# ug93tad/singa

Hardware: AMD Instinct MI355X
Metric: images/sec (whole node) ResNet-50 bf16 training (higher is better)
Workload: dtype bf16; 1 GPU; model=ResNet-50, global_batch=1024, image=224, parallelism=dp1, exec=hipgraph, optimizer=SGD momentum 0.9 wd 1e-4, deterministic=True

## Files before the change

### singa_amd/csrc/kernels/igemm.hip

```cpp
#include <stdio.h>
#include <stdlib.h>

#include <stdexcept>
#include <type_traits>

#include "igemm_kern.h"

namespace sg {

constexpr int WDOT_RB = 64;
__global__ void __launch_bounds__(256) wdot_colsum_k(const bf16* __restrict__ w, const float* __restrict__ dw,
                                                     int rows, int C, float sign, float* __restrict__ wdot,
                                                     const float* __restrict__ gamma, const float* __restrict__ beta,
                                                     float tau, int* __restrict__ flag) {
  __shared__ float red[4][64];
  const int cl = threadIdx.x & 63, lane = threadIdx.x >> 6;
  const int c = blockIdx.x * 64 + cl;
  if (gamma != nullptr && blockIdx.y == 0 && lane == 0 && c < C) {
    const float g = fabsf(gamma[c]);
    if (!(g >= tau && fabsf(beta[c]) <= 4.f * g)) *flag = 1;
  }
  const int r0 = blockIdx.y * WDOT_RB;
  float a = 0.f;
  if (c < C) {
    const int r1 = min(rows, r0 + WDOT_RB);
    for (int r = r0 + lane; r < r1; r += 4) a += (float)w[(int64_t)r * C + c] * dw[(int64_t)r * C + c];
  }
  red[lane][cl] = a;
  __syncthreads();
  if (lane == 0 && c < C) atomicAdd(wdot + c, sign * (red[0][cl] + red[1][cl] + red[2][cl] + red[3][cl]));
}

__global__ void __launch_bounds__(256) wt_transpose_k(const bf16* __restrict__ w, bf16* __restrict__ wt, int K,
                                                      int T, int C) {
  __shared__ bf16 tile[64][65];
  const int c0 = blockIdx.x * 64, k0 = blockIdx.y * 64, t = blockIdx.z;
  const int tx = threadIdx.x & 63, ty = threadIdx.x >> 6;
  for (int r = ty; r < 64; r += 4) {
    const int k = k0 + r, c = c0 + tx;
    tile[r][tx] = (k < K && c < C) ? w[((int64_t)k * T + t) * C + c] : (bf16)0.f;
  }
  __syncthreads();
  for (int r = ty; r < 64; r += 4) {
    const int c = c0 + r, k = k0 + tx;
    if (c < C && k < K) wt[((int64_t)t * C + c) * K + k] = tile[tx][r];
  }
}

struct WtDesc {
  const bf16* src;
  bf16* dst;
  int K, T, C, tile0;
};
__global__ void __launch_bounds__(256) wt_transpose_batched_k(const WtDesc* __restrict__ desc, int n) {
  __shared__ bf16 tile[64][65];
  int d = 0;
  while (d + 1 < n && desc[d + 1].tile0 <= (int)blockIdx.x) ++d;
  const WtDesc w = desc[d];
  const int lt = blockIdx.x - w.tile0;
  const int cb = (w.C + 63) / 64, kbn = (w.K + 63) / 64;
  const int c0 = (lt % cb) * 64, k0 = ((lt / cb) % kbn) * 64, t = lt / (cb * kbn);
  const int tx = threadIdx.x & 63, ty = threadIdx.x >> 6;
  for (int r = ty; r < 64; r += 4) {
    const int k = k0 + r, c = c0 + tx;
    tile[r][tx] = (k < w.K && c < w.C) ? w.src[((int64_t)k * w.T + t) * w.C + c] : (bf16)0.f;
  }
  __syncthreads();
  for (int r = ty; r < 64; r += 4) {
    const int c = c0 + r, k = k0 + tx;
    if (c < w.C && k < w.K) w.dst[((int64_t)t * w.C + c) * w.K + k] = tile[tx][r];
  }
}

}

using namespace sg;

static void init_phase_identity(ConvGeom& g) {
  for (int i = 0; i < 16; ++i) {
    g.phs[i].dns = FastDiv(1);
    g.phs[i].dWp = FastDiv(1);
    g.phs[i].dHpWp = FastDiv(1);
  }
}

static ConvGeom make_geom(int N, int H, int W, int C, int K, int R, int S, int Ho, int Wo, int sh, int sw, int ph,
                          int pw, int dh, int dw) {
  ConvGeom g{};
  g.N = N; g.H = H; g.W = W; g.C = C; g.K = K; g.R = R; g.S = S; g.Ho = Ho; g.Wo = Wo;
  g.sh = sh; g.sw = sw; g.ph = ph; g.pw = pw; g.dh = dh; g.dw = dw;
  g.dC = FastDiv(C); g.dS = FastDiv(S); g.dK = FastDiv(K); g.dWo = FastDiv(Wo); g.dHoWo = FastDiv(Ho * Wo);
  g.bq_n = BK / (Ho * Wo);
  g.bq_h = (BK % (Ho * Wo)) / Wo;
  g.bq_w = BK % Wo;
  init_phase_identity(g);
  return g;
}

static int make_phases(ConvGeom& g) {
  int np = 0;
  for (int a = 0; a < g.sh; ++a)
    for (int b = 0; b < g.sw; ++b) {
      Phase& P = g.phs[np++];
      P.a = a; P.b = b;
      P.r0 = (a + g.ph) % g.sh;
      P.s0 = (b + g.pw) % g.sw;
      P.nr = P.r0 < g.R ? (g.R - P.r0 + g.sh - 1) / g.sh : 0;
      P.ns = P.s0 < g.S ? (g.S - P.s0 + g.sw - 1) / g.sw : 0;
      P.offh = (a + g.ph - P.r0) / g.sh;
      P.offw = (b + g.pw - P.s0) / g.sw;
      P.Hp = a < g.H ? (g.H - a + g.sh - 1) / g.sh : 0;
      P.Wp = b < g.W ? (g.W - b + g.sw - 1) / g.sw : 0;
      P.dns = FastDiv(P.ns > 0 ? P.ns : 1);
      P.dWp = FastDiv(P.Wp > 0 ? P.Wp : 1);
      P.dHpWp = FastDiv(P.Hp * P.Wp > 0 ? P.Hp * P.Wp : 1);
    }
  return np;
}

extern "C" int sg_bn_deterministic();
static int g_tune[20] = {5, 1, 1, 0, 0, 1, 2, 1, 0, 1, 0, 0, 0, 1, 0, 1, 0, 0, 1, 0};
static thread_local int g_wt_ready = 0;
static thread_local const bf16* g_res_g = nullptr;
static thread_local int g_res_s = 1, g_res_Ho = 0, g_res_Wo = 0;
static thread_local const uint8_t* g_res_mask = nullptr;
static thread_local int g_mask_out = 0;

static int gemm_log() {
  static int on = [] {
    const char* e = getenv("SG_GEMM_LOG");
    return e && e[0] == '1' ? 1 : 0;
  }();
  return on;
}

constexpr int stages_c(int BM, int BN, int STAGES) { return STAGES * (BM + BN) * BK * 2; }

template <int BM, int BN, int AM, int BMODE, int OUT, int NTH = NT, int WM = 2, int WN = 2, int STAGES = 2,
          int FLAGS = 0>
static void launch_t(const GemmArgs& p_in, int tiles, int ydim, int zdim, hipStream_t s) {
  GemmArgs p = p_in;
  p.lds_epilogue = g_tune[1];
  p.epi_fence = g_tune[19];
  p.early_issue = g_tune[7];
  p.nt_store = g_tune[8];
  p.xcd_split = (OUT == OUT_F32_ATOMIC && g_tune[2] && ydim == 1 && zdim >= 8 && (zdim & 7) == 0) ? 1 : 0;
  dim3 grid(tiles, ydim, zdim), block(NTH);
  constexpr int stages = STAGES * (BM + BN) * BK * 2;
  constexpr int rch = (STAGES == 1 || BM * (BN + 4) * 4 <= 152 * 1024) ? BM : BM / 4;
  constexpr int etile = STAGES == 1 ? (OUT == OUT_BF16 ? BM * (BN + 8) * 2 : BM * (BN + 4) * 4)
                        : OUT == OUT_BF16 ? rch * (BN + 4) * 4
                        : OUT == OUT_F32_ATOMIC ? BM * (BN + 4) * 4 : 0;
  constexpr int ered = (OUT == OUT_BF16) ? NTH * 16 * 4 : 0;
  static_assert(STAGES != 1 || (OUT == OUT_BF16 && ered <= (etile > stages_c(BM, BN, STAGES) ? etile : stages_c(BM, BN, STAGES))),
                "single-stage variant: bf16 output only");
  constexpr int lds = stages > etile ? stages : etile;
  static_assert(lds <= 160 * 1024, "LDS budget");
  auto* kern = igemm_k<BM, BN, AM, BMODE, OUT, NTH, WM, WN, STAGES, FLAGS>;
  if (gemm_log())
    fprintf(stderr, "SG_GEMM_L igemm_k<%d,%d,%d,%d,%d,%d,%d,%d,%d,%d> grid %d %d %d\n", BM, BN, AM, BMODE, OUT, NTH, WM,
            WN, STAGES, FLAGS, tiles, ydim, zdim);
  if constexpr (lds > 65536) {
    static bool attr = [kern] {
      return hipFuncSetAttribute((const void*)kern, hipFuncAttributeMaxDynamicSharedMemorySize, lds) == hipSuccess;
    }();
    (void)attr;
  }
  hipLaunchKernelGGL(kern, grid, block, lds, s, p);
}

template <int OUT, int FLAGS = 0>
static void launch_pp(const GemmArgs& p_in, int tiles, int ydim, hipStream_t s) {
  GemmArgs p = p_in;
  p.lds_epilogue = g_tune[1];
  p.epi_fence = g_tune[19];
  p.nt_store = g_tune[8];
  constexpr int lds = 2 * PP_BUF;
  auto* kern = pp_gemm_k<OUT, FLAGS>;
  if (gemm_log()) fprintf(stderr, "SG_GEMM_L pp_gemm_k<%d,%d> grid %d %d 1\n", OUT, FLAGS, tiles, ydim);
  static bool attr = [kern] {
    return hipFuncSetAttribute((const void*)kern, hipFuncAttributeMaxDynamicSharedMemorySize, lds) == hipSuccess;
  }();
  (void)attr;
  hipLaunchKernelGGL(kern, dim3(tiles, ydim, 1), dim3(512), lds, s, p);
}

template <int KT, int EPI = 0, int AM = LM_KMAJOR>
static void launch_sk(const GemmArgs& p, int tiles_m, int tiles_n, hipStream_t s) {
  constexpr int lds = sk_lds(KT);
  auto* kern = sk_gemm_k<KT, EPI, AM>;
  static bool attr = [kern] {
    return hipFuncSetAttribute((const void*)kern, hipFuncAttributeMaxDynamicSharedMemorySize, lds) == hipSuccess;
  }();
  (void)attr;
  const int cus = sg_cu_count();
  int g = (cus + tiles_n - 1) / tiles_n;
  g = (g + 7) / 8 * 8;
  if (g > tiles_m) g = tiles_m >= 8 ? tiles_m / 8 * 8 : 8;
  GemmArgs q = p;
  q.wq = 8 * tiles_n <= QMAX ? sg_workq_slot() : nullptr;
  if (gemm_log())
    fprintf(stderr, "SG_GEMM_L sk_gemm_k<%d,%d,%d> grid %d %d 1 M=%d N=%d K=%d\n", KT, EPI, AM, g, tiles_n, p.M, p.N,
            p.K);
  hipLaunchKernelGGL(kern, dim3(g, tiles_n, 1), dim3(256), lds, s, q);
}

static void launch_st(const GemmArgs& p, int tiles_m, int tiles_n, hipStream_t s) {
  auto* kern = st_gemm_k<0>;
  static bool attr = [kern] {
    return hipFuncSetAttribute((const void*)kern, hipFuncAttributeMaxDynamicSharedMemorySize, ST_LDS) == hipSuccess;
  }();
  (void)attr;
  const int cus = sg_cu_count();
  int g = (cus + tiles_n - 1) / tiles_n;
  g = (g + 7) / 8 * 8;
  if (g > tiles_m) g = tiles_m >= 8 ? tiles_m / 8 * 8 : 8;
  GemmArgs q = p;
  q.wq = 8 * tiles_n <= QMAX ? sg_workq_slot() : nullptr;
  if (gemm_log())
    fprintf(stderr, "SG_GEMM_L st_gemm_k<0> grid %d %d 1 M=%d N=%d K=%d\n", g, tiles_n, p.M, p.N, p.K);
  hipLaunchKernelGGL(kern, dim3(g, tiles_n, 1), dim3(256), ST_LDS, s, q);
}

static int pick_big(int M, int N) {
  if (g_tune[4] == 5) return 1;
  if (g_tune[4] == 6) return 2;
  if (g_tune[4] == 7) return 3;
  if (g_tune[4] == 8) return 4;
  if (!g_tune[5] || g_tune[4] != 0) return 0;
  auto wg = [&](int bm, int bn) { return (long)((M + bm - 1) / bm) * ((N + bn - 1) / bn); };
  if (N >= 128 && !((N % 128) != 0 && (N % 128) <= 64) && wg(128, 128) >= 512) return 1;
  return 0;
}
static int big_bm(int big) { return big == 1 ? 128 : 256; }

static void pick_tile(int M, int N, int& BM, int& BN) {
  auto wg = [&](int bm, int bn) { return (long)((M + bm - 1) / bm) * ((N + bn - 1) / bn); };
  BM = 128;
  BN = N <= 64 ? 64 : 128;
  if (BN == 128 && (N % 128) != 0 && (N % 128) <= 64) BN = 64;
  if (wg(BM, BN) < 256 && M > 64) BM = 64;
  if (wg(BM, BN) < 256 && BN == 128) BN = 64;
}

template <int AM, int BMODE, int OUT>
static void launch_tile(const GemmArgs& p, int M, int BM, int BN, int splits, hipStream_t s, int batch, int zdim) {
  const int tiles = ((M + BM - 1) / BM) * ((p.N + BN - 1) / BN);
  const int z = zdim > 0 ? zdim : splits;
  if (BM == 128 && BN == 128) launch_t<128, 128, AM, BMODE, OUT>(p, tiles, batch, z, s);
  else if (BM == 128 && BN == 64) launch_t<128, 64, AM, BMODE, OUT>(p, tiles, batch, z, s);
  else if (BM == 64 && BN == 128) launch_t<64, 128, AM, BMODE, OUT>(p, tiles, batch, z, s);
  else launch_t<64, 64, AM, BMODE, OUT>(p, tiles, batch, z, s);
}

static void pick_wgrad(int M, int N, int K, int mode, int& BM, int& BN, int& splits) {
  const int nkt = (K + BK - 1) / BK;
  if (mode == 4) mode = ((long)K >= 8L * M * N) ? 1 : 0;
  if (mode == 0) {
    pick_tile(M, N, BM, BN);
    const int tiles = ((M + BM - 1) / BM) * ((N + BN - 1) / BN);
    splits = 1;
    while (tiles * splits < 768 && splits * 2 <= nkt / 4) splits *= 2;
    return;
  }
  auto fit = [](int d) { return (d >= 128 && !((d % 128) != 0 && (d % 128) <= 64)) ? 128 : 64; };
  BM = fit(M);
  BN = fit(N);
  const int tiles = ((M + BM - 1) / BM) * ((N + BN - 1) / BN);
  const int target = mode == 1 ? 512 : mode == 2 ? 1024 : 768;
  const int min_kt = mode == 2 ? 4 : 8;
  splits = 1;
  while (tiles * splits < target && (splits * 2) * min_kt <= nkt) splits *= 2;
}

template <int AM, int BMODE, int OUT, int FLAGS = 0>
static void launch(const GemmArgs& p, int M, int splits, hipStream_t s, int batch, int zdim) {
  int BM, BN;
  if (gemm_log())
    fprintf(stderr, "SG_GEMM am=%d bm=%d out=%d flags=%d M=%d N=%d K=%d splits=%d batch=%d z=%d beta=%g stats=%d "
                    "smode=%d det=%d res=%d bias=%d relu=%d act=%d phase=%d R=%d S=%d C=%d sh=%d\n",
            AM, BMODE, OUT, FLAGS, M, p.N, p.K, splits, batch, zdim, p.beta, p.stats != nullptr, p.stats_mode,
            p.stats_det, p.res_g != nullptr, p.bias != nullptr, p.relu, p.act, p.out_phase, p.g.R, p.g.S, p.g.C,
            p.g.sh);
  if constexpr (OUT != OUT_F32_ATOMIC) {
    {
      const int z = zdim > 0 ? zdim : 1;
      if (FLAGS == 0 && OUT == OUT_BF16 && AM == LM_KMAJOR && BMODE == LM_KMAJOR && g_tune[9] && g_tune[4] == 0 &&
          !p.out_phase && zdim <= 1 && batch == 1 && p.K <= 128 && (p.N & 127) == 0 && !p.bias && !p.relu &&
          p.alpha == 1.f && p.stats_mode == 0 && !(p.stats && p.stats_det) && g_tune[1] && !p.res_g &&
          (p.ldc & 7) == 0 && (long)((M + 127) / 128) * (p.N / 128) >= 2048) {
        const int tiles_m = (M + 127) / 128;
        if (p.K <= 64) launch_sk<1>(p, tiles_m, p.N / 128, s);
        else launch_sk<2>(p, tiles_m, p.N / 128, s);
        return;
      }
      if (FLAGS == 0 && OUT == OUT_BF16 && AM == LM_KMAJOR && BMODE == LM_KMAJOR && g_tune[18] && g_tune[4] == 0 &&
          (g_tune[18] >= 2 || p.K == 256 || (p.K == 512 && p.N == 128)) &&
          !p.out_phase && zdim <= 1 && batch == 1 && p.K >= 256 && (p.K & 63) == 0 && (p.N & 127) == 0 &&
          !p.bias && !p.relu && p.act == 0 && p.act_bwd == 0 && p.alpha == 1.f && p.beta == 0.f &&
          p.stats_mode == 0 && !(p.stats && p.stats_det) && !p.res_g && g_tune[1] && (p.ldc & 7) == 0 &&
          (p.lda & 7) == 0 && (p.ldb & 7) == 0 && (long)((M + 127) / 128) * (p.N / 128) >= 2048) {
        launch_st(p, (M + 127) / 128, p.N / 128, s);
        return;
      }
      int kmax = p.K;
      if (p.out_phase) {
        kmax = 0;
        for (int i = 0; i < z; ++i) kmax = max(kmax, p.g.phs[i].nr * p.g.phs[i].ns * p.g.K);
      }
      if (OUT == OUT_BF16 && g_tune[6] > 0 && g_tune[4] == 0 && p.beta == 0.f &&
          (kmax + BK - 1) / BK <= g_tune[6] && p.N >= 128 && !((p.N % 128) != 0 && (p.N % 128) <= 64) &&
          (long)((M + 127) / 128) * ((p.N + 127) / 128) >= 1024 && (g_tune[11] == 0 || !p.out_phase)) {
        const int tiles = ((M + 127) / 128) * ((p.N + 127) / 128);
        launch_t<128, 128, AM, BMODE, OUT_BF16, 256, 2, 2, 1, FLAGS>(p, tiles, batch, z, s);
        return;
      }
      int big = pick_big(M, p.N);
      const bool pp_ok = AM == LM_KMAJOR && BMODE == LM_KMAJOR && !p.out_phase && zdim <= 1 &&
                         !(p.stats && p.stats_det);
      if (big == 0 && g_tune[4] == 0 && g_tune[5] && pp_ok && p.K >= 2048 &&
          (long)((M + 255) / 256) * ((p.N + 255) / 256) >= 256)
        big = 4;
      if (big == 4) {
        if (pp_ok) {
          launch_pp<OUT, FLAGS>(p, ((M + 255) / 256) * ((p.N + 255) / 256), batch, s);
          return;
        }
        big = 1;
      }
      if (big == 1 && g_tune[16] > 0 && !sg_bn_deterministic() && M >= 256 &&
          (g_tune[16] >= 3 || AM == LM_CONV_FWD || (g_tune[16] == 2 && AM == LM_DGRAD_A)))
        big = 3;
      if (big == 1) {
        const int tiles = ((M + 127) / 128) * ((p.N + 127) / 128);
        launch_t<128, 128, AM, BMODE, OUT, 512, 2, 4, 2, FLAGS>(p, tiles, batch, z, s);
        return;
      }
      if (big == 2) {
        const int tiles = ((M + 255) / 256) * ((p.N + 63) / 64);
        launch_t<256, 64, AM, BMODE, OUT, 512, 4, 2, 4, FLAGS>(p, tiles, batch, z, s);
        return;
      }
      if (big == 3) {
        const int tiles = ((M + 255) / 256) * ((p.N + 127) / 128);
        launch_t<256, 128, AM, BMODE, OUT, 512, 4, 2, 3, FLAGS>(p, tiles, batch, z, s);
        return;
      }
    }
  }
  pick_tile(M, p.N, BM, BN);
  if (g_tune[4] > 0 && g_tune[4] < 5) {
    BM = (g_tune[4] == 2 || g_tune[4] == 3) ? 64 : 128;
    BN = (g_tune[4] == 1 || g_tune[4] == 3) ? 64 : 128;
  }
  const int tiles = ((M + BM - 1) / BM) * ((p.N + BN - 1) / BN);
  const int z = zdim > 0 ? zdim : splits;
  if constexpr ((AM == LM_KMAJOR || AM == LM_KOUTER) && (BMODE == LM_KMAJOR || BMODE == LM_KOUTER) && FLAGS == 0) {
    const long wgs = (long)tiles * (batch > 0 ? batch : 1) * (z > 0 ? z : 1);
    const int nkt = ((z > 1 ? p.k_per_split : p.K) + BK - 1) / BK;
    const bool ring = g_tune[14] == 3 || (g_tune[14] == 0 && wgs <= 4L * sg_cu_count() && nkt >= 8 && nkt <= 64);
    if (ring && !p.out_phase) {
      if (BM == 128 && BN == 128) launch_t<128, 128, AM, BMODE, OUT, NT, 2, 2, 3>(p, tiles, batch, z, s);
      else if (BM == 128 && BN == 64) launch_t<128, 64, AM, BMODE, OUT, NT, 2, 2, 3>(p, tiles, batch, z, s);
      else if (BM == 64 && BN == 128) launch_t<64, 128, AM, BMODE, OUT, NT, 2, 2, 3>(p, tiles, batch, z, s);
      else launch_t<64, 64, AM, BMODE, OUT, NT, 2, 2, 3>(p, tiles, batch, z, s);
      return;
    }
  }
  if (BM == 128 && BN == 128) launch_t<128, 128, AM, BMODE, OUT, NT, 2, 2, 2, FLAGS>(p, tiles, batch, z, s);
  else if (BM == 128 && BN == 64) launch_t<128, 64, AM, BMODE, OUT, NT, 2, 2, 2, FLAGS>(p, tiles, batch, z, s);
  else if (BM == 64 && BN == 128) launch_t<64, 128, AM, BMODE, OUT, NT, 2, 2, 2, FLAGS>(p, tiles, batch, z, s);
  else launch_t<64, 64, AM, BMODE, OUT, NT, 2, 2, 2, FLAGS>(p, tiles, batch, z, s);
}

static int pick_splits(int M, int N, int K, int want) {
  if (want > 0) return want;
  int BM, BN;
  pick_tile(M, N, BM, BN);
  const int tiles = ((M + BM - 1) / BM) * ((N + BN - 1) / BN);
  int splits = 1;
  const int nkt = (K + BK - 1) / BK;
  const int cap = 2 * sg_cu_count();
  while (tiles * splits * 2 <= cap && nkt / (splits * 2) >= 32) splits *= 2;
  if (tiles < cap / 8)
    while (tiles * splits < cap && nkt / (splits * 2) >= 4) splits *= 2;
  return splits;
}

static inline int kps(int K, int splits) {
  const int nkt = (K + BK - 1) / BK;
  return ((nkt + splits - 1) / splits) * BK;
}

static unsigned extent_bytes(int64_t elems) {
  if (elems * 2 >= (int64_t)1 << 31)
    throw std::runtime_error("igemm: operand exceeds 2 GiB (32-bit buffer offsets); split the batch");
  return (unsigned)(elems * 2);
}

extern "C" {

int sg_bn_deterministic();
int sg_ws_prezeroed();
int sg_conv3x3_ok(int N, int H, int W, int C, int K);
int sg_conv3x3_64(const void* x, const void* w, int wmode, void* y, void* stats, const void* mask, int N, int H,
                  int W, int C, int K, hipStream_t s);

void sg_gemm_heads(const void* a, int64_t lda, int a_kouter, const void* b, int64_t ldb, int b_kouter, void* c,
                   int64_t ldc, int M, int N, int K, float alpha, float beta, const void* bias, int relu,
                   int out_mode, int splits, int batch, int64_t sa, int64_t sb, int64_t sc, int bh, int64_t sa2,
                   int64_t sb2, int64_t sc2, hipStream_t s);

void sg_gemm(const void* a, int64_t lda, int a_kouter, const void* b, int64_t ldb, int b_kouter, void* c,
             int64_t ldc, int M, int N, int K, float alpha, float beta, const void* bias, int relu, int out_mode,
             int splits, int batch, int64_t sa, int64_t sb, int64_t sc, hipStream_t s) {
  sg_gemm_heads(a, lda, a_kouter, b, ldb, b_kouter, c, ldc, M, N, K, alpha, beta, bias, relu, out_mode, splits,
                batch, sa, sb, sc, 0, 0, 0, 0, s);
}

int sg_gemm_act(const void* a, int64_t lda, int a_kouter, const void* b, int64_t ldb, int b_kouter, void* c,
                int64_t ldc, int M, int N, int K, float alpha, const void* bias, int batch, int64_t sa, int64_t sb,
                int64_t sc, int act, void* aux, int act_bwd, const void* act_x, float* colsum, hipStream_t s) {
  if ((N & 7) != 0 || (ldc & 7) != 0 || !g_tune[1] || g_tune[4] != 0 || (act == 0) == (act_x == nullptr) ||
      M <= 0 || K <= 0 || batch != 1 || (colsum && (act != 0 || sg_bn_deterministic())))
    return 0;
  GemmArgs p{};
  init_phase_identity(p.g);
  p.sa = sa; p.sb = sb; p.sc = sc;
  p.M = M; p.N = N; p.K = K; p.a = (const bf16*)a; p.lda = lda; p.b = (const bf16*)b; p.ldb = ldb;
  p.c = c; p.ldc = ldc; p.alpha = alpha; p.beta = 0.f; p.bias = (const float*)bias; p.relu = 0;
  p.act = act; p.aux = (bf16*)aux; p.act_x = (const bf16*)act_x; p.act_bwd = act_bwd;
  if (colsum) {
    p.stats = colsum;
    p.stats_mode = 5;
    p.stats_det = 0;
  }
  p.k_per_split = kps(K, 1);
  p.a_bytes = extent_bytes(a_kouter ? (int64_t)(K - 1) * lda + M : (int64_t)(M - 1) * lda + K);
  p.b_bytes = extent_bytes(b_kouter ? (int64_t)(K - 1) * ldb + N : (int64_t)(N - 1) * ldb + K);
// ... 224 lines not shown
    if (wt && (K & 63) == 0) {
      if (!wt_ready)
        hipLaunchKernelGGL(wt_transpose_k, dim3((C + 63) / 64, (K + 63) / 64, 1), dim3(256), 0, s, (const bf16*)w,
                           (bf16*)wt, K, 1, C);
      p.b = (const bf16*)wt; p.ldb = K;
      if (p.stats && p.stats_mode == 4 && p.res_s <= 1 && out_mode == OUT_BF16 && beta == 0.f && g_tune[9] &&
          g_tune[4] == 0 && K <= 128 && (C & 127) == 0 && (long)((p.M + 127) / 128) * (C / 128) >= 2048) {
        GemmArgs q = p;
        q.ep_res = p.res_g;
        q.ep_mask = (uint8_t*)p.bnb_mask;
        q.res_g = nullptr;
        if (K <= 64) launch_sk<1, 2>(q, (p.M + 127) / 128, C / 128, s);
        else launch_sk<2, 2>(q, (p.M + 127) / 128, C / 128, s);
        return;
      }
      if (out_mode == OUT_F32) launch<LM_KMAJOR, LM_KMAJOR, OUT_F32>(p, p.M, 1, s, 1, 0);
      else launch<LM_KMAJOR, LM_KMAJOR, OUT_BF16>(p, p.M, 1, s, 1, 0);
    } else {
      p.b = (const bf16*)w; p.ldb = C;
      if (out_mode == OUT_F32) launch<LM_KMAJOR, LM_KOUTER, OUT_F32>(p, p.M, 1, s, 1, 0);
      else launch<LM_KMAJOR, LM_KOUTER, OUT_BF16>(p, p.M, 1, s, 1, 0);
    }
    return;
  }
  const int np = make_phases(p.g);
  int Mmax = 0;
  for (int i = 0; i < np; ++i) Mmax = Mmax > N * p.g.phs[i].Hp * p.g.phs[i].Wp ? Mmax : N * p.g.phs[i].Hp * p.g.phs[i].Wp;
  p.M = Mmax; p.N = C; p.K = R * S * K;
  p.a = (const bf16*)dy; p.lda = 0; p.b = (const bf16*)w; p.ldb = 0;
  p.c = dx; p.ldc = C; p.alpha = 1.f; p.beta = beta; p.bias = nullptr; p.relu = 0;
  p.out_phase = 1;
  p.k_per_split = kps(p.K, 1);
  p.a_bytes = extent_bytes((int64_t)N * Ho * Wo * K);
  p.b_bytes = extent_bytes((int64_t)K * R * S * C);
  extent_bytes((int64_t)N * H * W * C);
  if (wt && (K & 63) == 0) {
    if (!wt_ready)
      hipLaunchKernelGGL(wt_transpose_k, dim3((C + 63) / 64, (K + 63) / 64, R * S), dim3(256), 0, s, (const bf16*)w,
                         (bf16*)wt, K, R * S, C);
    p.b = (const bf16*)wt;
    if (out_mode == OUT_F32) launch<LM_DGRAD_A, LM_DGRAD_BT, OUT_F32>(p, Mmax, 1, s, 1, np);
    else launch<LM_DGRAD_A, LM_DGRAD_BT, OUT_BF16>(p, Mmax, 1, s, 1, np);
    return;
  }
  if (out_mode == OUT_F32) launch<LM_DGRAD_A, LM_DGRAD_B, OUT_F32>(p, Mmax, 1, s, 1, np);
  else launch<LM_DGRAD_A, LM_DGRAD_B, OUT_BF16>(p, Mmax, 1, s, 1, np);
}

static int wgrad_splits_q(int tiles, int nkt, int sp0, int per_cu = 2) {
  const int slots = per_cu * sg_cu_count();
  constexpr int e = 6;
  int best = sp0;
  long best_cost = (long)((tiles * sp0 + slots - 1) / slots) * ((nkt + sp0 - 1) / sp0 + e);
  for (int sp = 1; sp <= 2 * sp0 && nkt / sp >= 16; ++sp) {
    const long cost = (long)((tiles * sp + slots - 1) / slots) * ((nkt + sp - 1) / sp + e);
    if (cost < best_cost || (cost == best_cost && sp < best)) {
      best = sp;
      best_cost = cost;
    }
  }
  return best;
}

void sg_conv_wgrad(const void* x, const void* dy, void* dw_out, int N, int H, int W, int C, int K, int R, int S,
                   int Ho, int Wo, int sh, int sw, int ph, int pw, int dh, int dw, int splits, hipStream_t s) {
  GemmArgs p{};
  p.g = make_geom(N, H, W, C, K, R, S, Ho, Wo, sh, sw, ph, pw, dh, dw);
  p.M = K; p.N = R * S * C; p.K = N * Ho * Wo;
  p.a = (const bf16*)dy; p.lda = K; p.b = (const bf16*)x; p.ldb = 0;
  p.c = dw_out; p.ldc = R * S * C; p.alpha = 1.f; p.beta = 0.f; p.bias = nullptr; p.relu = 0;
  p.a_bytes = extent_bytes((int64_t)N * Ho * Wo * K);
  p.b_bytes = extent_bytes((int64_t)N * H * W * C);
  int BM, BN, sp;
  int mode = g_tune[0], extra = g_tune[3];
  if (mode == 5) {
    if (R * S > 1) {
      mode = 4;
      extra += K <= 128 ? 2 : 1;
    } else {
      mode = (sh > 1 || sw > 1 || C == 2 * K) ? 1 : 4;
    }
  }
  pick_wgrad(p.M, p.N, p.K, mode, BM, BN, sp);
  if (extra > 0) {
    const int nkt = (p.K + BK - 1) / BK;
    for (int i = 0; i < extra && sp * 2 <= nkt; ++i) sp *= 2;
  }
  const bool big = g_tune[5] && p.M >= 128 && p.N >= 128 && splits <= 0 && !sg_bn_deterministic();
  if (big) {
    const int tiles = ((p.M + 127) / 128) * ((p.N + 127) / 128);
    const int nkt = (p.K + BK - 1) / BK;
    const int target = g_tune[10] > 0 ? g_tune[10] : R * S > 1 ? 1024 : 512;
    sp = 1;
    while (tiles * sp < target && sp * 2 * 4 <= nkt) sp *= 2;
    if (g_tune[13] && g_tune[10] <= 0) sp = wgrad_splits_q(tiles, nkt, sp);
    if (g_tune[12] > 0) sp = g_tune[12];
    if (g_tune[15] == 1 && p.M >= 256 && (p.M & 255) == 0) {
      const int t2 = ((p.M + 255) / 256) * ((p.N + 127) / 128);
      int sp2 = 1;
      while (t2 * sp2 < target && sp2 * 2 * 4 <= nkt) sp2 *= 2;
      if (g_tune[13] && g_tune[10] <= 0) sp2 = wgrad_splits_q(t2, nkt, sp2, 1);
      if (g_tune[12] > 0) sp2 = g_tune[12];
      p.k_per_split = kps(p.K, sp2);
      launch_t<256, 128, LM_KOUTER, LM_WGRAD_B, OUT_F32_ATOMIC, 512, 4, 2, 3>(p, t2, 1, sp2, s);
      return;
    }
    if (g_tune[15] == 1 && g_tune[17] == 1 && p.M < 256 && p.N >= 256) {
      const int t2 = ((p.M + 127) / 128) * ((p.N + 255) / 256);
      int sp2 = 1;
      while (t2 * sp2 < target && sp2 * 2 * 4 <= nkt) sp2 *= 2;
      if (g_tune[13] && g_tune[10] <= 0) sp2 = wgrad_splits_q(t2, nkt, sp2, 1);
      if (g_tune[12] > 0) sp2 = g_tune[12];
      p.k_per_split = kps(p.K, sp2);
      launch_t<128, 256, LM_KOUTER, LM_WGRAD_B, OUT_F32_ATOMIC, 512, 2, 4, 3>(p, t2, 1, sp2, s);
      return;
    }
    p.k_per_split = kps(p.K, sp);
    launch_t<128, 128, LM_KOUTER, LM_WGRAD_B, OUT_F32_ATOMIC, 512, 2, 4, 2>(p, tiles, 1, sp, s);
    return;
  }
  if (splits > 0) sp = splits;
  if (sg_bn_deterministic()) sp = 1;
  p.k_per_split = kps(p.K, sp);
  launch_tile<LM_KOUTER, LM_WGRAD_B, OUT_F32_ATOMIC>(p, p.M, BM, BN, sp, s, 1, 0);
}

int sg_conv_stats_rows(int M, int N) {
  if ((N & 7) != 0 || !g_tune[1]) return 0;
  if (!sg_bn_deterministic()) return 32;
  if (int big = pick_big(M, N)) {
    if (big == 4) big = 1;
    return (M + big_bm(big) - 1) / big_bm(big);
  }
  int BM, BN;
  pick_tile(M, N, BM, BN);
  return (M + BM - 1) / BM;
}

void sg_set_wt_ready(int on) { g_wt_ready = on; }
void sg_set_dgrad_mask_out(int on) { g_mask_out = on; }
void sg_wdot_colsum(const void* w, const void* dw, int rows, int C, float sign, void* wdot, int zero_first,
                    const void* gamma, const void* beta, float tau, hipStream_t s) {
  if (zero_first && !sg_ws_prezeroed()) sg_zero_async(wdot, sizeof(float) * (C + 1), s);
  hipLaunchKernelGGL(wdot_colsum_k, dim3((C + 63) / 64, (rows + WDOT_RB - 1) / WDOT_RB), dim3(256), 0, s,
                     (const bf16*)w, (const float*)dw, rows, C, sign, (float*)wdot, (const float*)gamma,
                     (const float*)beta, tau, (int*)((float*)wdot + C));
}
void sg_wt_transpose_batched(const void* desc, int n, int total, hipStream_t s) {
  static_assert(sizeof(WtDesc) == 32, "descriptor layout shared with the Python packer");
  if (n > 0 && total > 0)
    hipLaunchKernelGGL(wt_transpose_batched_k, dim3(total), dim3(256), 0, s, (const WtDesc*)desc, n);
}
void sg_set_tuning(int key, int value) {
  if (key >= 0 && key < 20) g_tune[key] = value;
}
int sg_get_tuning(int key) { return key >= 0 && key < 20 ? g_tune[key] : 0; }

}
```

### singa_amd/csrc/kernels/igemm_kern.h

```cpp
#pragma once
#include <stdexcept>
#include <type_traits>

#include "common.h"

namespace sg {

constexpr int BK = 64, NT = 256;

enum LoadMode : int {
  LM_KMAJOR = 0,
  LM_KOUTER = 1,
  LM_CONV_FWD = 2,
  LM_DGRAD_A = 3,
  LM_WGRAD_B = 4,
  LM_DGRAD_B = 5,
  LM_DGRAD_BT = 6,
  LM_KMAJOR2 = 7,
  LM_KOUTER2 = 8,
};
enum OutMode : int { OUT_BF16 = 0, OUT_F32 = 1, OUT_F32_ATOMIC = 2 };

struct Phase {
  int a, b;
// ... 977 lines not shown
      else if constexpr (EPI == 2) wait_vmcnt<5 * NPS + D + 1>();
      else if (has_beta) wait_vmcnt<2 * NPS + D + 1>(); else wait_vmcnt<NPS + D + 1>();
    } else {
      if constexpr (EPI >= 1) wait_vmcnt<6 * NPS + D + 1>();
      else if (has_beta) wait_vmcnt<4 * NPS + D + 1>(); else wait_vmcnt<2 * NPS + D + 1>();
    }
    raw_barrier();
    f32x4 acc[TM][TN];
#pragma unroll
    for (int i = 0; i < TM; ++i)
#pragma unroll
      for (int j = 0; j < TN; ++j) acc[i][j] = f32x4{0.f, 0.f, 0.f, 0.f};
#pragma unroll
    for (int kt = 0; kt < KT; ++kt) {
      const char* a_img = sA + (buf * KT + kt) * SK_TILE;
      const char* b_img = sB + kt * SK_TILE;
#pragma unroll
      for (int kk = 0; kk < 2; ++kk) {
        bf16x8 fa[TM], fb[TN];
#pragma unroll
        for (int i = 0; i < TM; ++i) fa[i] = la.frag_at(a_img, oa0[i][kk], oa1[i][kk]);
#pragma unroll
        for (int j = 0; j < TN; ++j) fb[j] = lb.frag_at(b_img, ob0[j][kk], ob1[j][kk]);
#pragma unroll
        for (int i = 0; i < TM; ++i)
#pragma unroll
          for (int j = 0; j < TN; ++j)
            acc[i][j] = __builtin_amdgcn_mfma_f32_16x16x32_bf16(fb[j], fa[i], acc[i][j], 0, 0, 0);
      }
    }
#pragma unroll
    for (int i = 0; i < TM; ++i) {
      const int ml = wm * WTM + i * 16 + (l & 15);
#pragma unroll
      for (int j = 0; j < TN; ++j) {
        const int nl = wn * WTN + j * 16 + (l >> 4) * 4;
        bf16x4 o;
        o[0] = (bf16)acc[i][j][0]; o[1] = (bf16)acc[i][j][1]; o[2] = (bf16)acc[i][j][2]; o[3] = (bf16)acc[i][j][3];
        *(bf16x4*)(sC + ml * SK_LDT + nl) = o;
      }
    }
    if (it > 0 && wid == 0 && l == 0) {
      if constexpr (EPI >= 1) wait_vmcnt<3 * NPS + D>();
      else if (has_beta) wait_vmcnt<2 * NPS + D>(); else wait_vmcnt<NPS + D>();
      *sQ =p.wq ? xcd + 8 * (3 * G8 + ticket) : tm + 16 * G8;
    }
    __builtin_amdgcn_s_waitcnt(0xC07F);
    raw_barrier();
    if (it > 0) t2 = __builtin_amdgcn_readfirstlane(*sQ);
    queue_op();
    {
      const bool live = t2 < tiles_m;
      la.init(p, (live ? t2 : tm) * BM, M, P, p.lda, p.a, p.a_bytes);
#pragma unroll
      for (int kt = 0; kt < KT; ++kt) la.issue(p, t2 * BM, M, kt * BK, K, P, sA + (buf * KT + kt) * SK_TILE, live);
    }
    const int m0 = tm * BM;
    const int rows = min(BM, M - m0);
    const __amdgpu_buffer_rsrc_t rc =
        p.c ? make_rsrc((const bf16*)p.c + (int64_t)m0 * p.ldc, (unsigned)((int64_t)rows * p.ldc * 2)) : rnull;
    u32x4 old[NPS];
    if constexpr (EPI == 1) {
      const __amdgpu_buffer_rsrc_t rmk = make_rsrc(p.ep_mask + (int64_t)m0 * (N >> 3), (unsigned)(rows * (N >> 3)));
#pragma unroll
      for (int pass = 0; pass < NPS; ++pass) {
        const int ml = r0 + pass * RPP;
        bf16x8 o = *(const bf16x8*)(sC + ml * SK_LDT + ch * 8);
        const bf16x8 rb = __builtin_bit_cast(bf16x8, rres[pass]);
        unsigned b = 0;
#pragma unroll
        for (int r = 0; r < 8; ++r) {
          o[r] = (bf16)fmaxf((float)o[r] * esc[r] + esf[r] + (float)rb[r], 0.f);
          b |= ((float)o[r] > 0.f ? 1u : 0u) << r;
        }
        __builtin_amdgcn_raw_buffer_store_b128(__builtin_bit_cast(u32x4, o), rc, (unsigned)((ml * (int)p.ldc + n) * 2),
                                               0, 0);
        __builtin_amdgcn_raw_buffer_store_b8((unsigned char)b, rmk, (unsigned)(ml * (N >> 3) + (n >> 3)), 0, 0);
      }
      load_res(t1);
    } else if constexpr (EPI == 2) {
#pragma unroll
      for (int pass = 0; pass < NPS; ++pass) {
        const int ml = r0 + pass * RPP;
        bf16x8 o = *(const bf16x8*)(sC + ml * SK_LDT + ch * 8);
        const bf16x8 rb = __builtin_bit_cast(bf16x8, rres[pass]);
#pragma unroll
        for (int r = 0; r < 8; ++r)
          o[r] = ((mres[pass] >> r) & 1u) != 0 ? (bf16)((float)o[r] + (float)rb[r]) : (bf16)0.f;
        __builtin_amdgcn_raw_buffer_store_b128(__builtin_bit_cast(u32x4, o), rc, (unsigned)((ml * (int)p.ldc + n) * 2),
                                               0, 0);
        if (ml < rows) {
#pragma unroll
          for (int r = 0; r < 8; ++r) st_s[r] += (float)o[r];
        }
      }
      load_res(t1);
    } else {
      if (has_beta) {
#pragma unroll
        for (int pass = 0; pass < NPS; ++pass)
          old[pass] = __builtin_amdgcn_raw_buffer_load_b128(rc, (unsigned)(((r0 + pass * RPP) * (int)p.ldc + n) * 2), 0, 0);
      }
#pragma unroll
      for (int pass = 0; pass < NPS; ++pass) {
        const int ml = r0 + pass * RPP;
        bf16x8 o = *(const bf16x8*)(sC + ml * SK_LDT + ch * 8);
        if (has_beta) {
          const bf16x8 ob = __builtin_bit_cast(bf16x8, old[pass]);
#pragma unroll
          for (int r = 0; r < 8; ++r) o[r] = (bf16)((float)o[r] + p.beta * (float)ob[r]);
        }
        __builtin_amdgcn_raw_buffer_store_b128(__builtin_bit_cast(u32x4, o), rc, (unsigned)((ml * (int)p.ldc + n) * 2),
                                               0, 0);
        if (p.stats && ml < rows) {
#pragma unroll
          for (int r = 0; r < 8; ++r) {
            const float f = (float)o[r];
            st_s[r] += f;
            st_q[r] += f * f;
          }
        }
      }
    }
    tm = t1;
    t1 = t2;
    if (tm >= tiles_m) break;
  }
  wait_vmcnt<0>();
  if (p.wq && threadIdx.x == 0) wq_done(p.wq, 8 * (int)gridDim.y);
  if (EPI != 1 && p.stats) {
    __syncthreads();
    float* red = (float*)smem;
#pragma unroll
    for (int r = 0; r < 8; ++r) {
      red[threadIdx.x * 16 + r] = st_s[r];
      red[threadIdx.x * 16 + 8 + r] = st_q[r];
    }
    __syncthreads();
    if (threadIdx.x < CPRW * 16) {
      const int c = threadIdx.x >> 4, r = threadIdx.x & 15;
      const int nn = n0 + c * 8;
      if (nn < N) {
        float a = red[c * 16 + r];
        for (int k = 1; k < RPP; ++k) a += red[(k * CPRW + c) * 16 + r];
        const int col = r < 8 ? nn + r : N + nn + (r - 8);
        atomicAdd(p.stats + (int64_t)(blockIdx.x & 31) * 2 * N + col, a);
      }
    }
  }
}

constexpr int ST_STAGE = 2 * SK_TILE;

__device__ __forceinline__ int wq_take_nowait(int* slot, int q) {
  int v;
  int* addr = slot + q * QSTRIDE;
  asm volatile("global_atomic_add %0, %1, %2, off sc0" : "=v"(v) : "v"(addr), "v"(1) : "memory");
  return v;
}
constexpr int ST_LDS = 3 * ST_STAGE + SK_STG;

template <int EPI = 0>
__global__ void __launch_bounds__(256, 1) st_gemm_k(const GemmArgs p) {
  extern __shared__ __attribute__((aligned(16))) char smem[];
  constexpr int BM = 128, BN = 128, NTH = 256, WN = 2, WTM = 64, WTN = 64, TM = 4, TN = 4;
  static_assert(EPI == 0, "plain output with optional BN statistics");
  bf16* sC = (bf16*)(smem + 3 * ST_STAGE);
  int* sQ = (int*)(smem + ST_LDS - 16);
  const int M = p.M, N = p.N, K = p.K;
  const int KT = K / BK;
  const int tiles_m = (M + BM - 1) / BM;
  const int n0 = blockIdx.y * BN;
  const int G = (int)gridDim.x, G8 = G >> 3, xcd = blockIdx.x & 7;
  const int qid = blockIdx.y * 8 + xcd;
  int tm = xcd + 8 * (blockIdx.x >> 3);
  int t1 = tm + 8 * G8, t2 = tm + 16 * G8;
  const Phase& P = p.g.phs[0];
  const int l = threadIdx.x & 63;
  const int wid = threadIdx.x >> 6;
  const int wm = wid / WN, wn = wid % WN;
  if (tm >= tiles_m) {
    if (p.wq && threadIdx.x == 0) wq_done(p.wq, 8 * (int)gridDim.y);
    return;
  }
  Loader<BM, LM_KMAJOR, NTH> la, la1;
  Loader<BN, LM_KMAJOR, NTH> lb;
  lb.init(p, n0, N, P, p.ldb, p.b, p.b_bytes);
  la.init(p, tm * BM, M, P, p.lda, p.a, p.a_bytes);
  la1.init(p, (t1 < tiles_m ? t1 : tm) * BM, M, P, p.lda, p.a, p.a_bytes);
  constexpr int LPT = Loader<BM, LM_KMAJOR, NTH>::VPT + Loader<BN, LM_KMAJOR, NTH>::VPT;
  constexpr int CPRW = BN / 8, RPP = NTH / CPRW, NPS = BM / RPP;
  constexpr int E_OPS = NPS + 1;
  static_assert(2 * LPT + E_OPS < 64, "vmcnt range");
  auto issue = [&](Loader<BM, LM_KMAJOR, NTH>& a, int t, int kt, int st) {
    char* base = smem + st * ST_STAGE;
    const bool live = t < tiles_m;
    a.issue(p, t * BM, M, kt * BK, K, P, base, live);
    lb.issue(p, n0, N, kt * BK, K, P, base + SK_TILE, live);
  };
  issue(la, tm, 0, 0);
  issue(la, tm, 1, 1);

  int oa0[TM][2], oa1[TM][2], ob0[TN][2], ob1[TN][2];
#pragma unroll
  for (int kk = 0; kk < 2; ++kk) {
#pragma unroll
    for (int i = 0; i < TM; ++i) la.frag_offsets(wm * WTM + i * 16, kk, oa0[i][kk], oa1[i][kk]);
#pragma unroll
    for (int j = 0; j < TN; ++j) lb.frag_offsets(wn * WTN + j * 16, kk, ob0[j][kk], ob1[j][kk]);
  }
  const int ch = threadIdx.x % CPRW, r0 = threadIdx.x / CPRW;
  const int n = n0 + ch * 8;
  float st_s[8], st_q[8];
#pragma unroll
  for (int r = 0; r < 8; ++r) { st_s[r] = 0.f; st_q[r] = 0.f; }
  const __amdgpu_buffer_rsrc_t rnull = make_rsrc(nullptr, 0);
  typedef unsigned u32x4 __attribute__((ext_vector_type(4)));
  int ticket = 0;
  int stage = 0;
  for (int it = 0;; ++it) {
    f32x4 acc[TM][TN];
#pragma unroll
    for (int i = 0; i < TM; ++i)
#pragma unroll
      for (int j = 0; j < TN; ++j) acc[i][j] = f32x4{0.f, 0.f, 0.f, 0.f};
    for (int kt = 0; kt < KT; ++kt) {
      if (it > 0 && kt < 2) wait_vmcnt<LPT + E_OPS>();
      else wait_vmcnt<LPT>();
      raw_barrier();
      {
        const int fill = stage == 0 ? 2 : stage - 1;
        if (kt + 2 < KT) issue(la, tm, kt + 2, fill);
        else issue(la1, t1, kt + 2 - KT, fill);
      }
      const char* a_img = smem + stage * ST_STAGE;
      const char* b_img = a_img + SK_TILE;
#pragma unroll
      for (int kk = 0; kk < 2; ++kk) {
        bf16x8 fa[TM], fb[TN];
#pragma unroll
        for (int i = 0; i < TM; ++i) fa[i] = la.frag_at(a_img, oa0[i][kk], oa1[i][kk]);
#pragma unroll
        for (int j = 0; j < TN; ++j) fb[j] = lb.frag_at(b_img, ob0[j][kk], ob1[j][kk]);
#pragma unroll
        for (int i = 0; i < TM; ++i)
#pragma unroll
          for (int j = 0; j < TN; ++j)
            acc[i][j] = __builtin_amdgcn_mfma_f32_16x16x32_bf16(fb[j], fa[i], acc[i][j], 0, 0, 0);
      }
      stage = stage == 2 ? 0 : stage + 1;
    }
#pragma unroll
    for (int i = 0; i < TM; ++i) {
      const int ml = wm * WTM + i * 16 + (l & 15);
#pragma unroll
      for (int j = 0; j < TN; ++j) {
        const int nl = wn * WTN + j * 16 + (l >> 4) * 4;
        bf16x4 o;
        o[0] = (bf16)acc[i][j][0]; o[1] = (bf16)acc[i][j][1]; o[2] = (bf16)acc[i][j][2]; o[3] = (bf16)acc[i][j][3];
        *(bf16x4*)(sC + ml * SK_LDT + nl) = o;
      }
    }
    if (it > 0 && wid == 0 && l == 0) {
      wait_vmcnt<2 * LPT>();
      *sQ = p.wq ? xcd + 8 * (3 * G8 + ticket) : tm + 16 * G8;
    }
    __builtin_amdgcn_s_waitcnt(0xC07F);
    raw_barrier();
    if (it > 0) t2 = __builtin_amdgcn_readfirstlane(*sQ);
    if (wid == 0 && p.wq) {
      if (l == 0) ticket = wq_take_nowait(p.wq, qid);
    } else {
      __builtin_amdgcn_raw_buffer_store_b32(0u, rnull, 0u, 0, 0);
    }
    const int m0 = tm * BM;
    const int rows = min(BM, M - m0);
    const __amdgpu_buffer_rsrc_t rc =
        make_rsrc((const bf16*)p.c + (int64_t)m0 * p.ldc, (unsigned)((int64_t)rows * p.ldc * 2));
#pragma unroll
    for (int pass = 0; pass < NPS; ++pass) {
      const int ml = r0 + pass * RPP;
      const bf16x8 o = *(const bf16x8*)(sC + ml * SK_LDT + ch * 8);
      __builtin_amdgcn_raw_buffer_store_b128(__builtin_bit_cast(u32x4, o), rc, (unsigned)((ml * (int)p.ldc + n) * 2),
                                             0, 0);
      if (p.stats && ml < rows) {
#pragma unroll
        for (int r = 0; r < 8; ++r) {
          const float f = (float)o[r];
          st_s[r] += f;
          st_q[r] += f * f;
        }
      }
    }
    tm = t1;
    t1 = t2;
    if (tm >= tiles_m) break;
    la = la1;
    la1.init(p, (t1 < tiles_m ? t1 : tm) * BM, M, P, p.lda, p.a, p.a_bytes);
  }
  wait_vmcnt<0>();
  if (p.wq && threadIdx.x == 0) wq_done(p.wq, 8 * (int)gridDim.y);
  if (p.stats) {
    __syncthreads();
    float* red = (float*)smem;
#pragma unroll
    for (int r = 0; r < 8; ++r) {
      red[threadIdx.x * 16 + r] = st_s[r];
      red[threadIdx.x * 16 + 8 + r] = st_q[r];
    }
    __syncthreads();
    if (threadIdx.x < CPRW * 16) {
      const int c = threadIdx.x >> 4, r = threadIdx.x & 15;
      const int nn = n0 + c * 8;
      if (nn < N) {
        float a = red[c * 16 + r];
        for (int k = 1; k < RPP; ++k) a += red[(k * CPRW + c) * 16 + r];
        const int col = r < 8 ? nn + r : N + nn + (r - 8);
        atomicAdd(p.stats + (int64_t)(blockIdx.x & 31) * 2 * N + col, a);
      }
    }
  }
}

}
```

Measured before the change: 16770 images/s.

## Add 256-row tile variant of streaming GEMM kernel for selected 1x1 conv shapes

Templates the persistent streaming GEMM kernel on tile height and adds a 256-row, 512-thread variant. It is enabled by default for a hardcoded list of large ResNet-50 1x1 conv shapes. To fit LDS, the epilogue stages output in the just-consumed pipeline stage and writes it in two halves. The aim is more reuse of the B tile per loaded A row and fewer tile iterations per CU. The cost is more LDS and registers, an extra barrier, and a shape whitelist that only fits this model. It also adds optional compile-time timestamp probes and makes the ticket wait explicit.

```diff
diff --git a/singa_amd/csrc/kernels/igemm.hip b/singa_amd/csrc/kernels/igemm.hip
--- a/singa_amd/csrc/kernels/igemm.hip
+++ b/singa_amd/csrc/kernels/igemm.hip
@@ -119,7 +119,7 @@
 }
 
 extern "C" int sg_bn_deterministic();
-static int g_tune[20] = {5, 1, 1, 0, 0, 1, 2, 1, 0, 1, 0, 0, 0, 1, 0, 1, 0, 0, 1, 0};
+static int g_tune[21] = {5, 1, 1, 0, 0, 1, 2, 1, 0, 1, 0, 0, 0, 1, 0, 1, 0, 0, 1, 0, 1};
 static thread_local int g_wt_ready = 0;
 static thread_local const bf16* g_res_g = nullptr;
 static thread_local int g_res_s = 1, g_res_Ho = 0, g_res_Wo = 0;
@@ -205,10 +205,13 @@
   hipLaunchKernelGGL(kern, dim3(g, tiles_n, 1), dim3(256), lds, s, q);
 }
 
+template <int BM = 128>
 static void launch_st(const GemmArgs& p, int tiles_m, int tiles_n, hipStream_t s) {
-  auto* kern = st_gemm_k<0>;
+  auto* kern = st_gemm_k<0, BM>;
+  constexpr int lds = st_lds(BM);
+  static_assert(lds <= 160 * 1024, "LDS budget");
   static bool attr = [kern] {
-    return hipFuncSetAttribute((const void*)kern, hipFuncAttributeMaxDynamicSharedMemorySize, ST_LDS) == hipSuccess;
+    return hipFuncSetAttribute((const void*)kern, hipFuncAttributeMaxDynamicSharedMemorySize, lds) == hipSuccess;
   }();
   (void)attr;
   const int cus = sg_cu_count();
@@ -218,8 +221,16 @@
   GemmArgs q = p;
   q.wq = 8 * tiles_n <= QMAX ? sg_workq_slot() : nullptr;
   if (gemm_log())
-    fprintf(stderr, "SG_GEMM_L st_gemm_k<0> grid %d %d 1 M=%d N=%d K=%d\n", g, tiles_n, p.M, p.N, p.K);
-  hipLaunchKernelGGL(kern, dim3(g, tiles_n, 1), dim3(256), ST_LDS, s, q);
+    fprintf(stderr, "SG_GEMM_L st_gemm_k<0%s> grid %d %d 1 M=%d N=%d K=%d\n", BM == 128 ? "" : ",256", g, tiles_n, p.M,
+            p.N, p.K);
+  hipLaunchKernelGGL(kern, dim3(g, tiles_n, 1), dim3(2 * BM), lds, s, q);
+}
+
+static bool st256_shape(int M, int N, int K) {
+  static const int won[][3] = {{802816, 512, 256}, {802816, 256, 512}, {200704, 1024, 512}, {3211264, 128, 256}};
+  for (const auto& w : won)
+    if (N == w[1] && K == w[2] && M >= w[0]) return true;
+  return false;
 }
 
 static int pick_big(int M, int N) {
@@ -285,6 +296,15 @@
   if constexpr (OUT != OUT_F32_ATOMIC) {
     {
       const int z = zdim > 0 ? zdim : 1;
+      if (FLAGS == 0 && OUT == OUT_BF16 && AM == LM_KMAJOR && BMODE == LM_KMAJOR && g_tune[20] && g_tune[4] == 0 &&
+          !p.out_phase && zdim <= 1 && batch == 1 && p.K >= 128 && (p.K & 63) == 0 && (p.N & 127) == 0 &&
+          !p.bias && !p.relu && p.act == 0 && p.act_bwd == 0 && p.alpha == 1.f && p.beta == 0.f &&
+          p.stats_mode == 0 && !(p.stats && p.stats_det) && !p.res_g && g_tune[1] && (p.ldc & 7) == 0 &&
+          (p.lda & 7) == 0 && (p.ldb & 7) == 0 &&
+          (g_tune[20] >= 2 || ((long)((M + 127) / 128) * (p.N / 128) >= 2048 && st256_shape(M, p.N, p.K)))) {
+        launch_st<256>(p, (M + 255) / 256, p.N / 128, s);
+        return;
+      }
       if (FLAGS == 0 && OUT == OUT_BF16 && AM == LM_KMAJOR && BMODE == LM_KMAJOR && g_tune[9] && g_tune[4] == 0 &&
           !p.out_phase && zdim <= 1 && batch == 1 && p.K <= 128 && (p.N & 127) == 0 && !p.bias && !p.relu &&
           p.alpha == 1.f && p.stats_mode == 0 && !(p.stats && p.stats_det) && g_tune[1] && !p.res_g &&
@@ -815,8 +835,8 @@
     hipLaunchKernelGGL(wt_transpose_batched_k, dim3(total), dim3(256), 0, s, (const WtDesc*)desc, n);
 }
 void sg_set_tuning(int key, int value) {
-  if (key >= 0 && key < 20) g_tune[key] = value;
-}
-int sg_get_tuning(int key) { return key >= 0 && key < 20 ? g_tune[key] : 0; }
-
-}
+  if (key >= 0 && key < 21) g_tune[key] = value;
+}
+int sg_get_tuning(int key) { return key >= 0 && key < 21 ? g_tune[key] : 0; }
+
+}
diff --git a/singa_amd/csrc/kernels/igemm_kern.h b/singa_amd/csrc/kernels/igemm_kern.h
--- a/singa_amd/csrc/kernels/igemm_kern.h
+++ b/singa_amd/csrc/kernels/igemm_kern.h
@@ -1153,21 +1153,42 @@
 
 constexpr int ST_STAGE = 2 * SK_TILE;
 
-__device__ __forceinline__ int wq_take_nowait(int* slot, int q) {
-  int v;
+__device__ __forceinline__ void wq_take_nowait(int* slot, int q, int& ticket) {
   int* addr = slot + q * QSTRIDE;
-  asm volatile("global_atomic_add %0, %1, %2, off sc0" : "=v"(v) : "v"(addr), "v"(1) : "memory");
-  return v;
+  asm volatile("global_atomic_add %0, %1, %2, off sc0" : "+v"(ticket) : "v"(addr), "v"(1) : "memory");
+}
+template <int N>
+__device__ __forceinline__ void wq_ticket_wait(int& ticket) {
+  static_assert(N >= 0 && N < 64, "vmcnt range");
+  asm volatile("s_waitcnt vmcnt(%1)" : "+v"(ticket) : "i"(N) : "memory");
 }
 constexpr int ST_LDS = 3 * ST_STAGE + SK_STG;
-
-template <int EPI = 0>
-__global__ void __launch_bounds__(256, 1) st_gemm_k(const GemmArgs p) {
+constexpr int st_stage(int bm) { return bm * BK * 2 + SK_TILE; }
+constexpr int st_lds(int bm) { return bm == 128 ? ST_LDS : 3 * st_stage(bm) + 16; }
+
+#ifdef SG_ST_STAMPS
+#define ST_STAMP(i)                                                 \
+  do {                                                              \
+    __builtin_amdgcn_sched_barrier(0);                              \
+    const unsigned long long t_ = __builtin_amdgcn_s_memtime();     \
+    stamp_acc[i] += t_ - stamp_t;                                   \
+    stamp_t = t_;                                                   \
+    __builtin_amdgcn_sched_barrier(0);                              \
+  } while (0)
+#else
+#define ST_STAMP(i) do {} while (0)
+#endif
+
+template <int EPI = 0, int BM = 128>
+__global__ void __launch_bounds__(2 * BM, 1) st_gemm_k(const GemmArgs p) {
   extern __shared__ __attribute__((aligned(16))) char smem[];
-  constexpr int BM = 128, BN = 128, NTH = 256, WN = 2, WTM = 64, WTN = 64, TM = 4, TN = 4;
+  constexpr int BN = 128, NTH = 2 * BM, WN = 2, WTM = 64, WTN = 64, TM = 4, TN = 4;
+  constexpr int A_IMG = BM * BK * 2, STAGE = st_stage(BM);
   static_assert(EPI == 0, "plain output with optional BN statistics");
-  bf16* sC = (bf16*)(smem + 3 * ST_STAGE);
-  int* sQ = (int*)(smem + ST_LDS - 16);
+  static_assert(BM == 128 || BM == 256, "tile rows");
+  static_assert(st_lds(BM) <= 160 * 1024, "LDS budget");
+  static_assert(BM == 128 || SK_STG <= STAGE, "a staged half fits the consumed stage");
+  int* sQ = (int*)(smem + st_lds(BM) - 16);
   const int M = p.M, N = p.N, K = p.K;
   const int KT = K / BK;
   const int tiles_m = (M + BM - 1) / BM;
@@ -1194,10 +1215,10 @@
   constexpr int E_OPS = NPS + 1;
   static_assert(2 * LPT + E_OPS < 64, "vmcnt range");
   auto issue = [&](Loader<BM, LM_KMAJOR, NTH>& a, int t, int kt, int st) {
-    char* base = smem + st * ST_STAGE;
+    char* base = smem + st * STAGE;
     const bool live = t < tiles_m;
     a.issue(p, t * BM, M, kt * BK, K, P, base, live);
-    lb.issue(p, n0, N, kt * BK, K, P, base + SK_TILE, live);
+    lb.issue(p, n0, N, kt * BK, K, P, base + A_IMG, live);
   };
   issue(la, tm, 0, 0);
   issue(la, tm, 1, 1);
@@ -1219,6 +1240,10 @@
   typedef unsigned u32x4 __attribute__((ext_vector_type(4)));
   int ticket = 0;
   int stage = 0;
+#ifdef SG_ST_STAMPS
+  unsigned long long stamp_acc[8] = {0, 0, 0, 0, 0, 0, 0, 0};
+  unsigned long long stamp_t = __builtin_amdgcn_s_memtime();
+#endif
   for (int it = 0;; ++it) {
     f32x4 acc[TM][TN];
 #pragma unroll
@@ -1226,16 +1251,20 @@
 #pragma unroll
       for (int j = 0; j < TN; ++j) acc[i][j] = f32x4{0.f, 0.f, 0.f, 0.f};
     for (int kt = 0; kt < KT; ++kt) {
+      ST_STAMP(5);
       if (it > 0 && kt < 2) wait_vmcnt<LPT + E_OPS>();
       else wait_vmcnt<LPT>();
+      ST_STAMP(0);
       raw_barrier();
+      ST_STAMP(1);
       {
         const int fill = stage == 0 ? 2 : stage - 1;
         if (kt + 2 < KT) issue(la, tm, kt + 2, fill);
         else issue(la1, t1, kt + 2 - KT, fill);
       }
-      const char* a_img = smem + stage * ST_STAGE;
-      const char* b_img = a_img + SK_TILE;
+      ST_STAMP(2);
+      const char* a_img = smem + stage * STAGE;
+      const char* b_img = a_img + A_IMG;
 #pragma unroll
       for (int kk = 0; kk < 2; ++kk) {
         bf16x8 fa[TM], fb[TN];
@@ -1243,53 +1272,77 @@
         for (int i = 0; i < TM; ++i) fa[i] = la.frag_at(a_img, oa0[i][kk], oa1[i][kk]);
 #pragma unroll
         for (int j = 0; j < TN; ++j) fb[j] = lb.frag_at(b_img, ob0[j][kk], ob1[j][kk]);
+#ifdef SG_ST_STAMPS
+        __builtin_amdgcn_s_waitcnt(0xC07F);
+#endif
+        ST_STAMP(3);
 #pragma unroll
         for (int i = 0; i < TM; ++i)
 #pragma unroll
           for (int j = 0; j < TN; ++j)
             acc[i][j] = __builtin_amdgcn_mfma_f32_16x16x32_bf16(fb[j], fa[i], acc[i][j], 0, 0, 0);
+        ST_STAMP(4);
       }
       stage = stage == 2 ? 0 : stage + 1;
-    }
-#pragma unroll
-    for (int i = 0; i < TM; ++i) {
-      const int ml = wm * WTM + i * 16 + (l & 15);
-#pragma unroll
-      for (int j = 0; j < TN; ++j) {
-        const int nl = wn * WTN + j * 16 + (l >> 4) * 4;
-        bf16x4 o;
-        o[0] = (bf16)acc[i][j][0]; o[1] = (bf16)acc[i][j][1]; o[2] = (bf16)acc[i][j][2]; o[3] = (bf16)acc[i][j][3];
-        *(bf16x4*)(sC + ml * SK_LDT + nl) = o;
-      }
-    }
-    if (it > 0 && wid == 0 && l == 0) {
-      wait_vmcnt<2 * LPT>();
-      *sQ = p.wq ? xcd + 8 * (3 * G8 + ticket) : tm + 16 * G8;
-    }
-    __builtin_amdgcn_s_waitcnt(0xC07F);
-    raw_barrier();
-    if (it > 0) t2 = __builtin_amdgcn_readfirstlane(*sQ);
-    if (wid == 0 && p.wq) {
-      if (l == 0) ticket = wq_take_nowait(p.wq, qid);
+#ifdef SG_ST_STAMPS
+      ++stamp_acc[6];
+#endif
+    }
+    constexpr int HALVES = BM / 128, HPS = NPS / HALVES;
+    bf16* sC;
+    if constexpr (BM == 128) {
+      sC = (bf16*)(smem + 3 * STAGE);
     } else {
-      __builtin_amdgcn_raw_buffer_store_b32(0u, rnull, 0u, 0, 0);
+      sC = (bf16*)(smem + (stage == 0 ? 2 : stage - 1) * STAGE);
+      raw_barrier();
     }
     const int m0 = tm * BM;
     const int rows = min(BM, M - m0);
     const __amdgpu_buffer_rsrc_t rc =
         make_rsrc((const bf16*)p.c + (int64_t)m0 * p.ldc, (unsigned)((int64_t)rows * p.ldc * 2));
 #pragma unroll
-    for (int pass = 0; pass < NPS; ++pass) {
-      const int ml = r0 + pass * RPP;
-      const bf16x8 o = *(const bf16x8*)(sC + ml * SK_LDT + ch * 8);
-      __builtin_amdgcn_raw_buffer_store_b128(__builtin_bit_cast(u32x4, o), rc, (unsigned)((ml * (int)p.ldc + n) * 2),
-                                             0, 0);
-      if (p.stats && ml < rows) {
-#pragma unroll
-        for (int r = 0; r < 8; ++r) {
-          const float f = (float)o[r];
-          st_s[r] += f;
-          st_q[r] += f * f;
+    for (int h = 0; h < HALVES; ++h) {
+      if (h > 0) raw_barrier();
+      if (HALVES == 1 || (wm >> 1) == h) {
+#pragma unroll
+        for (int i = 0; i < TM; ++i) {
+          const int ml = (wm & 1) * WTM + i * 16 + (l & 15);
+#pragma unroll
+          for (int j = 0; j < TN; ++j) {
+            const int nl = wn * WTN + j * 16 + (l >> 4) * 4;
+            bf16x4 o;
+            o[0] = (bf16)acc[i][j][0]; o[1] = (bf16)acc[i][j][1]; o[2] = (bf16)acc[i][j][2]; o[3] = (bf16)acc[i][j][3];
+            *(bf16x4*)(sC + ml * SK_LDT + nl) = o;
+          }
+        }
+      }
+      if (h == 0 && it > 0 && wid == 0 && l == 0) {
+        wq_ticket_wait<2 * LPT>(ticket);
+        *sQ = p.wq ? xcd + 8 * (3 * G8 + ticket) : tm + 16 * G8;
+      }
+      __builtin_amdgcn_s_waitcnt(0xC07F);
+      raw_barrier();
+      if (h == 0) {
+        if (it > 0) t2 = __builtin_amdgcn_readfirstlane(*sQ);
+        if (wid == 0 && p.wq) {
+          if (l == 0) wq_take_nowait(p.wq, qid, ticket);
+        } else {
+          __builtin_amdgcn_raw_buffer_store_b32(0u, rnull, 0u, 0, 0);
+        }
+      }
+#pragma unroll
+      for (int pass = 0; pass < HPS; ++pass) {
+        const int ml = r0 + pass * RPP, mg = h * 128 + ml;
+        const bf16x8 o = *(const bf16x8*)(sC + ml * SK_LDT + ch * 8);
+        __builtin_amdgcn_raw_buffer_store_b128(__builtin_bit_cast(u32x4, o), rc,
+                                               (unsigned)((mg * (int)p.ldc + n) * 2), 0, 0);
+        if (p.stats && mg < rows) {
+#pragma unroll
+          for (int r = 0; r < 8; ++r) {
+            const float f = (float)o[r];
+            st_s[r] += f;
+            st_q[r] += f * f;
+          }
         }
       }
     }
@@ -1300,6 +1353,14 @@
     la1.init(p, (t1 < tiles_m ? t1 : tm) * BM, M, P, p.lda, p.a, p.a_bytes);
   }
   wait_vmcnt<0>();
+#ifdef SG_ST_STAMPS
+  if (l == 0 && p.ep_mask) {
+    unsigned long long* o =
+        (unsigned long long*)p.ep_mask + ((int64_t)(blockIdx.y * gridDim.x + blockIdx.x) * (NTH / 64) + wid) * 8;
+#pragma unroll
+    for (int i = 0; i < 8; ++i) o[i] = stamp_acc[i];
+  }
+#endif
   if (p.wq && threadIdx.x == 0) wq_done(p.wq, 8 * (int)gridDim.y);
   if (p.stats) {
     __syncthreads();
```

Result: no change. 16830 images/s, median of 6 (+0.4%).
